# pzou01/unitree-rl-gym

Measured on AMD Instinct MI355X. Metric: env-steps/sec + PPO-iter wall-time, Go2 4096 envs/GPU at 1/2/4/8 MI355X, higher is better.
Workload: dtype fp32 env step; bf16 MFMA policy GEMMs (fp32 accumulate); 1 GPU; Go2 flat terrain, 4096 envs/GPU, MLP actor-critic 512-256-128, PPO 24 steps x 5 epochs x 4 mini-batches; num_envs_per_gpu=4096, decimation=4, parallelism=dp1

## Files before the change

unitree-rl-gym_amd/csrc/leggedsim.hip:

```cpp
#include <hip/hip_runtime.h>

#include <algorithm>
#include <cfloat>
#include <cmath>
#include <cstdint>
#include <cstdio>
#include <cstdlib>
#include <cstring>
#include <string>
#include <vector>

#include "../../include/leggedsim.h"
#include "lgs_detmath.h"

#define LGS_NPHASE 32
#ifdef LGS_PHASE_STAMPS
__device__ unsigned long long* g_phase_buf;
#define STAMP(i)                                                                                 \
    do {                                                                                         \
        __builtin_amdgcn_sched_barrier(0);                                                       \
        unsigned long long _t;                                                                   \
        asm volatile("s_memtime %0\n\ts_waitcnt lgkmcnt(0)" : "=s"(_t)::"memory");             \
        __builtin_amdgcn_sched_barrier(0);                                                       \
        if (threadIdx.x == 0) {                                                                  \
            if ((i) > 0) s.stamps[(i)] += _t - s.tlast;                                          \
            s.tlast = _t;                                                                        \
        }                                                                                        \
    } while (0)
#define STAMP_FLUSH(e)                                                                           \
    do {                                                                                         \
        if (threadIdx.x < LGS_NPHASE && g_phase_buf)                                             \
            g_phase_buf[(size_t)(e) * LGS_NPHASE + threadIdx.x] = s.stamps[threadIdx.x];         \
    } while (0)
#define STAMP_INIT()                                                                             \
    do {                                                                                         \
        if (threadIdx.x < LGS_NPHASE) s.stamps[threadIdx.x] = 0;                                 \
        if (threadIdx.x == 0) {                                                                  \
            s.stamps[18] = _wt0; s.stamps[20] = _wr0;                                            \
            s.stamps[22] = _whw; s.stamps[23] = _wxcc;                                           \
        }                                                                                        \
    } while (0)
#define STAMP_BEGIN()                                                                            \
    unsigned long long _wt0, _wr0;                                                               \
    unsigned _whw, _wxcc;                                                                        \
    asm volatile("s_memtime %0\n\ts_memrealtime %1\n\ts_getreg_b32 %2, hwreg(HW_REG_HW_ID)\n\t"   \
                 "s_getreg_b32 %3, hwreg(HW_REG_XCC_ID)\n\ts_waitcnt lgkmcnt(0)"                    \
                 : "=s"(_wt0), "=s"(_wr0), "=s"(_whw), "=s"(_wxcc)::"memory")
#define STAMP_END()                                                                              \
    do {                                                                                         \
        unsigned long long _t, _r;                                                               \
        asm volatile("s_memtime %0\n\ts_memrealtime %1\n\ts_waitcnt lgkmcnt(0)"                    \
                     : "=s"(_t), "=s"(_r)::"memory");                                            \
        if (threadIdx.x == 0) { s.stamps[19] = _t; s.stamps[21] = _r; }                          \
    } while (0)
#else
#define STAMP_BEGIN() do {} while (0)
#define STAMP_END() do {} while (0)
#define STAMP(i) do {} while (0)
#define STAMP_FLUSH(e) do {} while (0)
#define STAMP_INIT() do {} while (0)
#endif
#ifndef LGS_WAVES_PER_EU
#define LGS_WAVES_PER_EU 4
#endif
#ifndef LGS_WAVES_PER_EU_48
#define LGS_WAVES_PER_EU_48 3
#endif
#define MAXB LGS_MAX_BODIES
#define MAXD LGS_MAX_DEPTH
#define LGS_MAX_CHUNKS 32
#define LGS_PREFILTER_MARGIN 1e-3f
#define WAVE 64
// ... 3 lines not shown
static int set_err(int code, const std::string& msg) {
    g_err = msg;
    return code;
}
#define HIP_TRY(x)                                                                        \
    do {                                                                                  \
        hipError_t _e = (x);                                                              \
        if (_e != hipSuccess) return set_err(LGS_ERR_HIP, std::string(#x ": ") + hipGetErrorString(_e)); \
    } while (0)

struct DevModel {
    int B, D, P;
    int Br, Dr;
    const int* parent;
    const int* dof;
    const int* subtree_end;
    const int* depth;
    const int* chain;
    const float* joint_rot;
    const float* joint_pos;
    const float* axis;
    const float* mass;
    const float* com;
    const float* inertia;
    const float* dof_lower;
    const float* dof_upper;
    const float* dof_velocity;
    const int* pt_body;
    const float* pt_pos;
    const float* pt_radius;
    const float* bsph;
    const unsigned* chunk32;
    int nch32;
};

struct DevSim {
    float dt, gx, gy, gz;
    int iters;
    float contact_offset, rest_offset, max_depen, beta, ground_friction, armature;
    int clamp_qd, max_contacts, max_rows;
    const int16_t* hf;
    int hf_rows, hf_cols;
    float hf_inv_hs, hf_vs, hf_border;
    float hf_slope1, hf_nmin;
    const float4* selfp;
    int n_selfp, max_self;
    unsigned long long* stats;
};

__device__ __forceinline__ void count_drops(const DevSim& sp, int lane, int k, int v) {
    if (lane == 0 && v > 0) atomicAdd(sp.stats + LGS_NUM_CONTACT_STATS * (blockIdx.x & 7u) + k, (unsigned long long)v);
}

struct DevState {
    float* root;
    float* dofs;
    float* cforce;
    float* rbs;
    const float* friction;
    const float* added_mass;
    const float* torques_in;
    float* vsim;
    unsigned* pushed;
};

__device__ __forceinline__ float rl(float x, int l) {
// ... 138 lines not shown
    const float a = dot3(d1, d1), e = dot3(d2, d2), f = dot3(d2, r);
    const float eps = 1e-12f;
    float s, t;
    if (a <= eps && e <= eps) {
        s = 0.f; t = 0.f;
    } else if (a <= eps) {
        s = 0.f; t = clipf(f / e, 0.f, 1.f);
    } else {
        const float c = dot3(d1, r);
        if (e <= eps) {
            t = 0.f; s = clipf(-c / a, 0.f, 1.f);
        } else {
            const float b = dot3(d1, d2);
            const float den = a * e - b * b;
            s = den != 0.f ? clipf((b * f - c * e) / den, 0.f, 1.f) : 0.f;
            t = (b * s + f) / e;
            if (t < 0.f) { t = 0.f; s = clipf(-c / a, 0.f, 1.f); }
            else if (t > 1.f) { t = 1.f; s = clipf((b - c) / a, 0.f, 1.f); }
        }
    }
#pragma unroll
    for (int k = 0; k < 3; ++k) { c1[k] = p1[k] + d1[k] * s; c2[k] = p2[k] + d2[k] * t; }
}
__device__ __forceinline__ void self_tangents(const float* n, float* t1, float* t2) {
    float a0, a1, a2;
    if (fabsf(n[0]) < 0.57735f) { a0 = 1.f - n[0] * n[0]; a1 = 0.f - n[0] * n[1]; a2 = 0.f - n[0] * n[2]; }
    else { a0 = 0.f - n[1] * n[0]; a1 = 1.f - n[1] * n[1]; a2 = 0.f - n[1] * n[2]; }
    const float inv = 1.f / sqrtf(a0 * a0 + a1 * a1 + a2 * a2);
    t1[0] = a0 * inv; t1[1] = a1 * inv; t1[2] = a2 * inv;
    cross3(n, t1, t2);
}

template <int D, int B>
struct ModelCache {
    int dof[B], depth[B], se[B], dofbody[D > 0 ? D : 1];
    unsigned anc[D > 0 ? D : 1];
    unsigned char chain[B][MAXD];
    float jr[B][9], jp[B][3], ax[B][3], com[B][3], mass[B], in[B][6];
    float lo[D > 0 ? D : 1], hi[D > 0 ? D : 1], vl[D > 0 ? D : 1];
    float bs[B][5];
    unsigned ch32[LGS_MAX_CHUNKS];
};

template <int EPW, int D, int B>
__device__ __forceinline__ unsigned chunk_bodies(const ModelCache<D, B>& mc, int ch) {
    return EPW == 2 ? mc.ch32[ch] : (mc.ch32[2 * ch] | mc.ch32[2 * ch + 1]);
}

enum {
    MI_LIN_VEL = 0,
    MI_ANG_VEL = 3,
    MI_GRAVITY = 6,
    MI_PHASE = 9,
    MI_LEG_PHASE = 10,
    MI_CMD = 12,
    MI_CLEARANCE = 16,
    MI_FOOT_GROUND = 17,
    MI_COUNT = MI_FOOT_GROUND + LGS_MAX_FEET
};

template <int D, int B, int ROWS>
struct Smem {
    static constexpr int n = 6 + D;
    static constexpr int NP = (n % 2 == 0) ? n + 1 : n;
    static constexpr int AS = (ROWS % 2 == 0) ? ROWS + 1 : ROWS;
    static constexpr int EL = (D > LGS_MAX_CONTACT_BODIES ? D : LGS_MAX_CONTACT_BODIES) | 1;
    float root[16];
// ... 18 lines not shown
            float misc[32];
            static_assert(MI_COUNT <= 32, "misc holds every MI_* slot");
            float el[LGS_MAX_REWARDS][EL];
        } post;
        struct {
            int pwin[B];
            int sec_body[ROWS / 4];
            float sec[ROWS / 4][7];
            int sc_ab[ROWS / 4][2];
            float sc_tmp[ROWS / 4][7];
        } sel;
    } u;
    static constexpr int LP = (n + 3) / 4 * 4;
    __attribute__((aligned(16))) float L[n][LP];
    float Linv[n];
    float qf[n];
    float tgt[ROWS];
    int c_body[ROWS / 3];
    int c_body2[ROWS / 3];
    float c_pt[ROWS / 3][3];
    float c_fr[ROWS / 3][9];
    float c_sep[ROWS / 3];
    float cf[B][3];
    int flags[8];
    struct {
        long long ep;
        float cmd[4];
        float last_act[D > 0 ? D : 1], last_qd[D > 0 ? D : 1];
        float air[LGS_MAX_FEET];
        int lastc[LGS_MAX_FEET];
        float sums[LGS_MAX_REWARDS + 1];
        float kp[D > 0 ? D : 1], kd[D > 0 ? D : 1], strength[D > 0 ? D : 1];
        int delay;
    } pre;
#ifdef LGS_PHASE_STAMPS
    unsigned long long stamps[LGS_NPHASE];
    unsigned long long tlast;
#endif
};

template <int D, int B>
__device__ __forceinline__ void load_model(ModelCache<D, B>& c, const DevModel& md) {
    const int lane = threadIdx.x;
    if (lane < B) {
        const int j = md.dof[lane];
        c.dof[lane] = j;
        c.depth[lane] = md.depth[lane];
        c.se[lane] = md.subtree_end[lane];
        c.mass[lane] = md.mass[lane];
        if (j >= 0) c.dofbody[j] = lane;
    }
    for (int i = lane; i < B * MAXD; i += WAVE) (&c.chain[0][0])[i] = (unsigned char)md.chain[i];
    for (int i = lane; i < 9 * B; i += WAVE) (&c.jr[0][0])[i] = md.joint_rot[i];
    for (int i = lane; i < 3 * B; i += WAVE) {
        (&c.jp[0][0])[i] = md.joint_pos[i];
        (&c.ax[0][0])[i] = md.axis[i];
        (&c.com[0][0])[i] = md.com[i];
    }
    for (int i = lane; i < 6 * B; i += WAVE) (&c.in[0][0])[i] = md.inertia[i];
    for (int i = lane; i < 5 * B; i += WAVE) (&c.bs[0][0])[i] = md.bsph[i];
    if (lane < LGS_MAX_CHUNKS) c.ch32[lane] = lane < md.nch32 ? md.chunk32[lane] : 0u;
    if (lane < D) {
        int bj = 0;
        for (int b = 0; b < B; ++b) bj = md.dof[b] == lane ? b : bj;
        unsigned am = 0u;
        for (int b = 0; b <= bj; ++b) {
            const int i = md.dof[b];
            if (i >= 0 && i <= lane && bj < md.subtree_end[b]) am |= 1u << i;
        }
        c.anc[lane] = am;
        c.lo[lane] = md.dof_lower[lane];
        c.hi[lane] = md.dof_upper[lane];
        c.vl[lane] = md.dof_velocity[lane];
    }
}

template <int D, int CH>
__host__ __device__ constexpr bool l_nz(int i, int k) {
    return CH == 0 || k >= D || i >= D || i <= k + (D - 1 - k) % CH;
}

template <int D, int CH, int n, int LP>
__device__ __forceinline__ void uniform_back(const float* b, const float (*L)[LP], const float* Linv, float* xv) {
#pragma unroll
    for (int i = 0; i < n; ++i) xv[i] = b[i];
#pragma unroll
    for (int i = n - 1; i >= 0; --i) {
        float t = xv[i];
#pragma unroll
        for (int k = n - 1; k > i; --k)
            if (l_nz<D, CH>(k, i)) t = fmaf(-L[k][i], xv[k], t);
        xv[i] = t * Linv[i];
    }
}
template <int D, int CH, int n, int LP>
__device__ __forceinline__ void uniform_solve(const float* b, const float (*L)[LP], const float* Linv, float* xv) {
    float yv[n];
#pragma unroll
    for (int i = 0; i < n; ++i) {
        float t = b[i];
#pragma unroll
        for (int k = 0; k < i; ++k)
            if (l_nz<D, CH>(i, k)) t = fmaf(-L[i][k], yv[k], t);
        yv[i] = t * Linv[i];
    }
#pragma unroll
    for (int i = n - 1; i >= 0; --i) {
        float t = yv[i];
#pragma unroll
        for (int k = n - 1; k > i; --k)
            if (l_nz<D, CH>(k, i)) t = fmaf(-L[k][i], xv[k], t);
        xv[i] = t * Linv[i];
    }
}

template <int D, int B, int ROWS, int CH, int EPW, bool PAD = false>
__device__ void substep(Smem<D, B, ROWS>* sm, const ModelCache<D, B>& mc, const DevModel& md, const DevSim& sp,
                        float added_mass, float shape_mu, bool want_cf) {
    constexpr int n = 6 + D;
    Smem<D, B, ROWS>& s = sm[hh<EPW>()];
    int lane = hl<EPW>();
    asm volatile("" : "+v"(lane));
    const float dt = sp.dt;
    const float idt = 1.0f / dt;

    STAMP(0);
    if (lane < D) axis_angle(mc.ax[mc.dofbody[lane]], s.q[lane], s.u.fk.Ra[lane]);
    __syncthreads();
    if (lane < B) {
        float R[9], p[3], aw[3] = {0.f, 0.f, 0.f};
        quat_to_mat(s.root + 3, R);
        p[0] = s.root[0]; p[1] = s.root[1]; p[2] = s.root[2];
        const int d = mc.depth[lane];
        for (int l = 1; l <= d; ++l) {
            const int a = mc.chain[lane][l];
            float Rj[9], t[3];
            matmul(R, mc.jr[a], Rj);
            matvec(R, mc.jp[a], t);
            p[0] += t[0]; p[1] += t[1]; p[2] += t[2];
            const int j = mc.dof[a];
            if (j >= 0) {
                if (l == d) matvec(Rj, mc.ax[a], aw);
                matmul(Rj, s.u.fk.Ra[j], R);
            } else {
#pragma unroll
                for (int k = 0; k < 9; ++k) R[k] = Rj[k];
            }
        }
        float c[3];
        matvec(R, mc.com[lane], c);
#pragma unroll
        for (int k = 0; k < 9; ++k) s.R[lane][k] = R[k];
#pragma unroll
        for (int k = 0; k < 3; ++k) {
            s.p[lane][k] = p[k];
            s.aw[lane][k] = aw[k];
            s.cw[lane][k] = p[k] + c[k];
        }
    }
// ... 891 lines not shown
            matmul(R, mc.jr[a], Rj);
            matvec(R, mc.jp[a], tp);
            p[0] += tp[0]; p[1] += tp[1]; p[2] += tp[2];
            const int j = mc.dof[a];
            if (j >= 0) {
                matvec(Rj, mc.ax[a], aw);
                float Ra[9];
                axis_angle(mc.ax[a], s.q[j], Ra);
                matmul(Rj, Ra, R);
                const float qd = s.qd[j];
                float rp[3] = {p[0] - O[0], p[1] - O[1], p[2] - O[2]}, sv[3];
                cross3(rp, aw, sv);
#pragma unroll
                for (int k = 0; k < 3; ++k) { Vw[k] += aw[k] * qd; Vv[k] += sv[k] * qd; }
            } else {
#pragma unroll
                for (int k = 0; k < 9; ++k) R[k] = Rj[k];
            }
        }
        float c[3];
        matvec(R, mc.com[lane], c);
        float r[3] = {p[0] + c[0] - O[0], p[1] + c[1] - O[1], p[2] + c[2] - O[2]}, wr[3];
        cross3(Vw, r, wr);
        float* o = rbs_out + 13 * lane;
        o[0] = p[0]; o[1] = p[1]; o[2] = p[2];
        float qq[4];
        mat_to_quat(R, qq);
        o[3] = qq[0]; o[4] = qq[1]; o[5] = qq[2]; o[6] = qq[3];
#pragma unroll
        for (int k = 0; k < 3; ++k) { o[7 + k] = Vv[k] + wr[k]; o[10 + k] = Vw[k]; }
    }
}

template <int D, int B, int ROWS, int EPW, bool PAD = false>
__device__ __forceinline__ void load_state(Smem<D, B, ROWS>& s, const DevState& st, const DevModel& md, int e) {
    const int Dr = PAD ? md.Dr : D;
    const int lane = hl<EPW>();
    if (lane < 13) s.root[lane] = st.root[13 * e + lane];
    if (lane < 2 * D) {
        const float v = lane < 2 * Dr ? st.dofs[(size_t)2 * Dr * e + lane] : 0.f;
        if (lane & 1) s.qd[lane >> 1] = v; else s.q[lane >> 1] = v;
    }
}
template <int D, int B, int ROWS, int EPW, bool PAD = false>
__device__ __forceinline__ void store_state(Smem<D, B, ROWS>& s, const DevState& st, const DevModel& md, int e) {
    int lane = hl<EPW>();
    asm volatile("" : "+v"(lane));
    if (lane < 13) st.root[13 * e + lane] = s.root[lane];
    const int Dr = PAD ? md.Dr : D, Br = PAD ? md.Br : B;
    if (lane < 2 * Dr) st.dofs[(size_t)2 * Dr * e + lane] = (lane & 1) ? s.qd[lane >> 1] : s.q[lane >> 1];
    for (int i = lane; i < 3 * Br; i += WAVE / EPW) st.cforce[(size_t)3 * Br * e + i] = (&s.cf[0][0])[i];
}

template <int D, int B, int ROWS, int EPW, bool PAD = false>
__device__ __forceinline__ void load_post_inputs(Smem<D, B, ROWS>& s, const lgs_task_params& T,
                                                 const lgs_env_buffers& E, int N, int e, bool post) {
    const int lane = hl<EPW>();
    const int A = T.num_actions, Ad = PAD ? A : D, nf = T.num_feet;
    if (!post) {
        if (lane < Ad) s.pre.last_qd[lane] = E.last_dof_vel[Ad * e + lane];
        return;
    }
    const int nsum = T.num_rewards + (T.has_termination_reward ? 1 : 0);
    const float la = E.last_actions[A * e + (lane < A ? lane : 0)];
    const float lq = E.last_dof_vel[Ad * e + (lane < Ad ? lane : 0)];
    const float cm = E.commands[4 * e + (lane & 3)];
    const float su = E.episode_sums[(size_t)(lane < nsum ? lane : 0) * N + e];
    const long long ep = E.episode_length[e];
    float air = 0.f;
    int lc = 0;
    if (nf > 0) {
        air = E.feet_air_time[nf * e + (lane < nf ? lane : 0)];
        lc = E.last_contacts[nf * e + (lane < nf ? lane : 0)];
    }
    if (lane < A) s.pre.last_act[lane] = la;
    if (lane < Ad) s.pre.last_qd[lane] = lq;
    if (lane < 4) s.pre.cmd[lane] = cm;
    if (lane < nsum) s.pre.sums[lane] = su;
    if (lane < nf) { s.pre.air[lane] = air; s.pre.lastc[lane] = lc; }
    if (lane == 0) s.pre.ep = ep;
}

template <int D, int B, int ROWS, int CH, bool PAD = false>
__global__ __launch_bounds__(WAVE) void k_simulate(DevModel md, DevSim sp, DevState st, int N) {
    __shared__ Smem<D, B, ROWS> s;
    __shared__ ModelCache<D, B> mc;
    const int e = xcd_env(blockIdx.x, gridDim.x);
    if (e >= N) return;
    load_model(mc, md);
    const int Dr = PAD ? md.Dr : D, Br = PAD ? md.Br : B;
    load_state<D, B, ROWS, 1, PAD>(s, st, md, e);
    if (threadIdx.x < D)
        s.tau[threadIdx.x] = threadIdx.x < Dr ? st.torques_in[(size_t)Dr * e + threadIdx.x] : 0.f;
    __syncthreads();
    substep<D, B, ROWS, CH, 1, PAD>(&s, mc, md, sp, st.added_mass ? st.added_mass[e] : 0.f, st.friction ? st.friction[e] : 1.f, true);
    store_state<D, B, ROWS, 1, PAD>(s, st, md, e);
    if (st.rbs) body_states<D, B, ROWS, 1>(s, mc, st.rbs + (size_t)13 * Br * e, Br);
}

template <int D, int B, int ROWS, int CH, bool PAD = false>
__global__ __launch_bounds__(WAVE) void k_fk(DevModel md, DevState st, int N) {
    __shared__ Smem<D, B, ROWS> s;
    __shared__ ModelCache<D, B> mc;
    const int e = xcd_env(blockIdx.x, gridDim.x);
    if (e >= N) return;
    load_model(mc, md);
    const int Br = PAD ? md.Br : B;
    load_state<D, B, ROWS, 1, PAD>(s, st, md, e);
    __syncthreads();
    body_states<D, B, ROWS, 1>(s, mc, st.rbs + (size_t)13 * Br * e, Br);
}

struct DevEnv {
// ... 255 lines not shown

struct TerrainTail {
    long long* levels;
    const long long* types;
    const float* origins;
    long long* level_sum;
    float* heights;
    float hf_hs;
    float hf_inv_hs, hf_vs, hf_border;
    const int16_t* hf;
    int hf_rows, hf_cols;
    int obs_scan;
    float obs_offset, obs_clip, obs_scale, obs_noise;
};
__device__ __forceinline__ const TerrainTail& terrain_tail(const lgs_task_params& T) {
    return *reinterpret_cast<const TerrainTail*>(&T + 1);
}
__global__ void k_set_terrain_tail(TerrainTail* dst, TerrainTail v) { *dst = v; }

struct ActuatorTail {
    float* kp_scale;
    float* kd_scale;
    float* strength;
    int* delay;
    int enabled, resample;
    float kp_lo, kp_hi, kd_lo, kd_hi, st_lo, st_hi;
    int dl_lo, dl_hi;
};
static_assert(sizeof(TerrainTail) % alignof(ActuatorTail) == 0, "ActuatorTail follows TerrainTail");
__device__ __forceinline__ const ActuatorTail& actuator_tail(const lgs_task_params& T) {
    return *reinterpret_cast<const ActuatorTail*>(&terrain_tail(T) + 1);
}

template <int D, int B, int ROWS, int EPW, bool PAD = false>
__device__ __forceinline__ void load_actuator(Smem<D, B, ROWS>& s, const lgs_task_params& T,
                                              const lgs_env_buffers& E, int e, bool post) {
    const int lane = hl<EPW>();
    const int A = T.num_actions;
    const ActuatorTail& X = actuator_tail(T);
    const int jd = lane < D ? lane : 0;
    float kp = T.p_gains[jd], kd = T.d_gains[jd], st = 1.f;
    int dl = 0;
    if (X.enabled) {
        const size_t r = (size_t)A * e + (lane < A ? lane : 0);
        const float ks = X.kp_scale[r], ds = X.kd_scale[r], m = X.strength[r];
        dl = X.delay[e];
        if (!post) {
            const float la = E.last_actions[r];
            if (lane < A) s.pre.last_act[lane] = la;
        }
        if (lane < A) { kp = (kp * ks) * m; kd = (kd * ds) * m; st = m; }
        if (PAD && lane >= A && lane < D) s.pre.last_act[lane] = 0.f;
    }
    if (lane < D) { s.pre.kp[lane] = kp; s.pre.kd[lane] = kd; s.pre.strength[lane] = st; }
    if (lane == 0) s.pre.delay = dl;
}

template <int EPW>
__device__ __forceinline__ void resample_actuator(const lgs_task_params& T, int e, uint32_t step) {
    const ActuatorTail& X = actuator_tail(T);
    if (!X.enabled || !X.resample) return;
    const int lane = hl<EPW>();
    const int A = T.num_actions;
    const uint64_t seed = T.seed;
    if (lane < A) {
        const size_t r = (size_t)A * e + lane;
        X.kp_scale[r] = rand_range(X.kp_lo, X.kp_hi, philox_uniform(seed, e, step, LGS_STREAM_ACTUATOR, lane));
        X.kd_scale[r] = rand_range(X.kd_lo, X.kd_hi, philox_uniform(seed, e, step, LGS_STREAM_ACTUATOR, LGS_MAX_DOFS + lane));
        X.strength[r] = rand_range(X.st_lo, X.st_hi, philox_uniform(seed, e, step, LGS_STREAM_ACTUATOR, 2 * LGS_MAX_DOFS + lane));
    }
    if (lane == 0) {
        const int n = X.dl_hi - X.dl_lo + 1;
        X.delay[e] = X.dl_lo + min((int)(philox_uniform(seed, e, step, LGS_STREAM_ACTUATOR, 3 * LGS_MAX_DOFS) * (float)n), n - 1);
    }
}
template <int EPW>
__device__ __forceinline__ void height_scan(const TerrainTail& sp, const lgs_task_params& T, const float* root,
                                            float* out) {
    const int lane = hl<EPW>();
    const int ny = T.num_height_y, P = T.num_height_x * ny;
    const float qz = root[5], qw = root[6];
    const float nq = sqrtf(qz * qz + qw * qw);
    const float z = qz / nq, w = qw / nq;
    const float c = w * w - z * z, sn = 2.f * w * z;
    const float bx = root[0], by = root[1];
    for (int k = lane; k < P; k += WAVE / EPW) {
        const int ix = k / ny, iy = k - ix * ny;
// ... 370 lines not shown
            rand_range(-T.max_push_vel_xy, T.max_push_vel_xy, philox_uniform(seed, e, step, LGS_STREAM_PUSH, lane));
    } else if (lane < 6) {
        E.last_root_vel[6 * e + lane] = s.root[7 + lane];
    }
    if (vsim && lane >= 2 && lane < 6) E.last_root_vel[6 * e + lane] = s.root[7 + lane];
}

enum { MODE_STEP = 0, MODE_PHYSICS = 1, MODE_POST = 2, MODE_POST_REWARDS = 3, MODE_POST_FINISH = 4,
       MODE_POST_PREPARE = 5, MODE_POST_TERM_REWARDS = 6 };
__host__ __device__ constexpr int mode_part(int mode) {
    return mode == MODE_POST_REWARDS ? PART_REWARDS
         : mode == MODE_POST_FINISH ? PART_FINISH
         : mode == MODE_POST_PREPARE ? PART_PREPARE
         : mode == MODE_POST_TERM_REWARDS ? PART_TERM_REWARDS : PART_ALL;
}

template <int D, int B, int ROWS, int CH, int EPW, int WPE = 0, bool PAD = false>
__global__ __launch_bounds__(WAVE) __attribute__((amdgpu_waves_per_eu(WPE > 0 ? WPE : (EPW == 2 ? 2 : (ROWS <= 32 ? LGS_WAVES_PER_EU : LGS_WAVES_PER_EU_48))))) void k_step(DevModel md, DevSim sp, DevState st, const lgs_task_params* __restrict__ Tp,
                                               lgs_env_buffers E, int N, uint32_t step, int mode) {
    STAMP_BEGIN();
    __shared__ Smem<D, B, ROWS> sm[EPW];
    __shared__ ModelCache<D, B> mc;
#ifndef LGS_PHASE_STAMPS
    static_assert(EPW != 2 || EPW * sizeof(Smem<D, B, ROWS>) + sizeof(ModelCache<D, B>) <= 20 * 1024,
                  "k_step: LDS per workgroup above 20 KB");
#endif
    if (E.step_counter) step = (uint32_t)*E.step_counter;
    if (blockIdx.x == 0 && threadIdx.x == 0 && st.pushed && mode != MODE_PHYSICS) st.pushed[2] = step;
    const int e = EPW * xcd_env(blockIdx.x, gridDim.x) + hh<EPW>();
    if (EPW * xcd_env(blockIdx.x, gridDim.x) >= N) return;
    Smem<D, B, ROWS>& s = sm[hh<EPW>()];
    const lgs_task_params& T = *Tp;
    const int lane = hl<EPW>();
    load_model(mc, md);
#ifdef LGS_DIAG_MULTISTEP
    const uint32_t step0 = step;
    for (int tt = 0; tt < LGS_DIAG_MULTISTEP; ++tt) {
    step = step0 + (uint32_t)tt;
    __syncthreads();
#endif
    load_state<D, B, ROWS, EPW, PAD>(s, st, md, e);
    load_post_inputs<D, B, ROWS, EPW, PAD>(s, T, E, N, e, mode != MODE_PHYSICS);
    const int A = T.num_actions;
    const int Ad = PAD ? A : D, Br = PAD ? md.Br : B;
    float* rbs = (T.write_body_states && st.rbs) ? st.rbs + (size_t)13 * Br * e : nullptr;
    STAMP_INIT();
    if (mode == MODE_STEP || mode == MODE_PHYSICS) {
        load_actuator<D, B, ROWS, EPW, PAD>(s, T, E, e, mode != MODE_PHYSICS);
        float a = 0.f;
        if (lane < A) {
            const float* ain = E.actions_in ? E.actions_in : E.actions;
            a = clipf(ain[A * e + lane], -T.clip_actions, T.clip_actions);
            E.actions[A * e + lane] = a;
            s.act[lane] = a;
        }
        const float am = st.added_mass ? st.added_mass[e] : 0.f;
        const float mu = st.friction ? st.friction[e] : 1.f;
        __syncthreads();
        float traw = 0.f;
        for (int it = 0; it < T.decimation; ++it) {
            if (lane < D) {
                const float as = (it < s.pre.delay ? s.pre.last_act[lane] : a) * T.action_scale;
                const float q = s.q[lane], qd = s.qd[lane];
                const float kp = s.pre.kp[lane], kd = s.pre.kd[lane];
                float t;
                if (T.control_type == 0 && T.clamp_pd_targets) {
                    const float tg = clipf(as + T.default_dof_pos[lane], T.pd_target_lower[lane], T.pd_target_upper[lane]);
                    t = kp * (tg - q) - kd * qd;
                }
                else if (T.control_type == 0) t = kp * (as + T.default_dof_pos[lane] - q) - kd * qd;
                else if (T.control_type == 1) {
                    const float lqd = lane < Ad ? s.pre.last_qd[lane] : 0.f;
                    t = kp * (as - qd) - kd * (qd - lqd) / sp.dt;
                }
                else t = as * s.pre.strength[lane];
                traw = t;
                s.tau[lane] = clipf(t, -T.torque_limits[lane], T.torque_limits[lane]);
            }
            __syncthreads();
#ifndef LGS_DIAG_IO_ONLY
            substep<D, B, ROWS, CH, EPW, PAD>(sm, mc, md, sp, am, mu, it == T.decimation - 1);
#else
            if (lane < 3 * B) (&s.cf[0][0])[lane] = 0.f;
#endif
        }
        STAMP(0);
        if (T.record_unclipped_torques) {
            __syncthreads();
            if (lane < D) s.tau[lane] = traw;
        }
        if (lane < Ad) E.torques[Ad * e + lane] = s.tau[lane];
        if (rbs) body_states<D, B, ROWS, EPW>(s, mc, rbs, Br, T.body_state_mask);
    } else {
        if (lane < A) s.act[lane] = E.actions[A * e + lane];
        if (lane < D) s.tau[lane] = lane < Ad ? E.torques[Ad * e + lane] : 0.f;
        for (int i = lane; i < 3 * B; i += WAVE / EPW)
            (&s.cf[0][0])[i] = i < 3 * Br ? st.cforce[(size_t)3 * Br * e + i] : 0.f;
    }
    __syncthreads();
    STAMP(15);
    if (mode != MODE_PHYSICS)
        post_physics<D, B, ROWS, EPW, PAD>(s, T, E, rbs, N, e, step, RESET_STEP, mode_part(mode), st.vsim, st.pushed);
    __syncthreads();
    STAMP(16);
    store_state<D, B, ROWS, EPW, PAD>(s, st, md, e);
    STAMP(17);
    STAMP_END();
    STAMP_FLUSH(e);
#ifdef LGS_DIAG_MULTISTEP
    }
// ... 48 lines not shown
        float m = E.ep_means[nsum];
        if (any) m = (float)*E.terrain_level_sum / (float)N;
        E.ep_means[nsum] = m;
        if (E.ep_snapshot) E.ep_snapshot[nsum] = m;
    }
    if (E.time_outs_carry && any)
        for (int e = t; e < N; e += blockDim.x) E.time_outs_carry[e] = E.time_out[e];
    __syncthreads();
    if (t <= nsum) E.episode_acc[t] = 0.f;
    if (E.episode_acc_next && t <= nsum) E.episode_acc_next[t] = 0.f;
    if (t == 0 && advance) pushed_flag[(step + 1u) & 1u] = 0u;
    if (t == 0 && E.step_counter && advance) *E.step_counter += 1;
}

__global__ void k_copy_rows(float* dst, const float* src, const int32_t* ids, int n, int width) {
    const int i = blockIdx.x * blockDim.x + threadIdx.x;
    const int row = i / width, col = i % width;
    if (row >= n) return;
    const size_t r = (size_t)ids[row];
    dst[r * width + col] = src[r * width + col];
}

struct Inst;
struct Kernels;
struct lgs_sim {
    int N, B, D, P;
    const Inst* inst = nullptr;
    const Kernels* kern = nullptr;
    int device;
    hipStream_t stream = nullptr;
    DevModel md{};
    DevSim sp{};
    void* model_mem = nullptr;
    float* friction = nullptr;
    float* added_mass = nullptr;
    float* vsim = nullptr;
    unsigned* pushed = nullptr;
    unsigned long long* stats = nullptr;
    float* root = nullptr;
    float* dofs = nullptr;
    float* cforce = nullptr;
    float* rbs = nullptr;
    const float* torques = nullptr;
    lgs_task_params* task_dev = nullptr;
    int16_t* hf_mem = nullptr;
    float4* self_mem = nullptr;
    int has_task = 0;
    int task_curriculum = 0, task_heights = 0;
    int task_obs = 0, task_priv = 0, task_layout = 0, task_actions = 0, task_scan = 0;
    lgs_height_obs hobs{};
    float hf_hs = 0.f;
    TerrainTail tail_host{};
    lgs_actuator_rand act{};
    int task_decimation = 0;
    int epw = 1;
    std::vector<std::string> body_names, dof_names;
};

#define LGS_ROBOT_SHAPES X(12, 13, 6) X(10, 11, 5) X(12, 19, 3)

#ifndef LGS_EXTRA_SHAPES
#define LGS_EXTRA_SHAPES X(23, 24)
#endif
#ifndef LGS_GENERIC_SHAPES
#define LGS_GENERIC_SHAPES X(16, 24) X(26, 32)
#endif

enum Fit {
    FIT_EXACT,
    FIT_BODIES,
    FIT_DOFS
};

struct Kernels {
    using Step = void (*)(DevModel, DevSim, DevState, const lgs_task_params*, lgs_env_buffers, int, uint32_t, int);
    Step step;
    Step step_small;
    Step step2;
    void (*simulate)(DevModel, DevSim, DevState, int);
    void (*fk)(DevModel, DevState, int);
    void (*reset_all)(DevModel, DevState, const lgs_task_params*, lgs_env_buffers, int, uint32_t, const uint8_t*);
};
template <int D, int B, int ROWS, int CH, bool PAD, bool EPW2>
static Kernels kernels_of() {
    Kernels k{};
    k.step = k_step<D, B, ROWS, CH, 1, PAD ? 2 : 0, PAD>;
    if constexpr (EPW2) k.step2 = k_step<D, B, ROWS, CH, 2, 0, PAD>;
    else if constexpr (!PAD) k.step_small = k_step<D, B, ROWS, CH, 1, 4, PAD>;
    k.simulate = k_simulate<D, B, ROWS, CH, PAD>;
    k.fk = k_fk<D, B, ROWS, CH, PAD>;
    k.reset_all = k_reset_all<D, B, ROWS, CH, PAD>;
    return k;
}

struct Inst {
    int Dt, Bt;
    int rows;
    int chain;
    Fit fit;
    bool epw2;
    Kernels chained, dense;
    bool takes(int D, int B) const {
        return fit == FIT_DOFS ? D <= Dt && B + (Dt - D) <= Bt : D == Dt && (fit == FIT_BODIES ? B <= Bt : B == Bt);
    }
};
template <int D, int B, int ROWS, int CH, Fit FIT, bool EPW2>
static Inst inst_of() {
    constexpr bool PAD = FIT != FIT_EXACT;
    return {D, B, ROWS, CH, FIT, EPW2, kernels_of<D, B, ROWS, CH, PAD, EPW2>(), kernels_of<D, B, ROWS, 0, PAD, EPW2>()};
}
static const Inst g_insts[] = {
#define X(D_, B_, CH_) inst_of<D_, B_, 32, CH_, FIT_EXACT, true>(),
    LGS_ROBOT_SHAPES
#undef X
#define X(D_, B_, CH_) inst_of<D_, B_, 48, CH_, FIT_EXACT, false>(),
    LGS_ROBOT_SHAPES
#undef X
#define X(D_, B_) inst_of<D_, B_, 48, 0, FIT_BODIES, false>(),
    LGS_EXTRA_SHAPES
#undef X
#define X(D_, B_) inst_of<D_, B_, 48, 0, FIT_DOFS, false>(),
    LGS_GENERIC_SHAPES
#undef X
};
// ... 136 lines not shown
    for (int b = B; b < Bt; ++b) bsph[(size_t)5 * b + 3] = -1.f;
    size_t ints = (size_t)Bt * (4 + LGS_MAX_DEPTH) + (size_t)P + chunk32.size();
    size_t floats = (size_t)Bt * (9 + 3 + 3 + 1 + 3 + 6 + 5) + (size_t)Dt * 3 + (size_t)P * 4;
    size_t bytes = ints * 4 + floats * 4 + 512;
    HIP_TRY(hipMalloc(&s->model_mem, bytes));
    char* host = (char*)calloc(1, bytes);
    size_t off = 0;
    auto put = [&](const void* src, size_t n) -> size_t {
        size_t o = off;
        if (n) memcpy(host + off, src, n);
        off += (n + 15) & ~size_t(15);
        return o;
    };
    size_t o_parent = put(parent.data(), 4 * Bt), o_dof = put(dofv.data(), 4 * Bt), o_se = put(se.data(), 4 * Bt);
    size_t o_depth = put(depth.data(), 4 * Bt), o_chain = put(chain.data(), 4 * Bt * LGS_MAX_DEPTH);
    size_t o_jr = put(jr.data(), 36 * Bt), o_jp = put(jp.data(), 12 * Bt), o_ax = put(ax.data(), 12 * Bt);
    size_t o_mass = put(mass.data(), 4 * Bt), o_com = put(com.data(), 12 * Bt), o_in = put(inertia.data(), 24 * Bt);
    size_t o_lo = put(dlo.data(), 4 * Dt), o_hi = put(dhi.data(), 4 * Dt), o_vel = put(dvel.data(), 4 * Dt);
    size_t o_pb = put(m->pt_body, 4 * P), o_pp = put(m->pt_pos, 12 * P), o_pr = put(m->pt_radius, 4 * P);
    size_t o_bs = put(bsph.data(), 20 * Bt), o_ch = put(chunk32.data(), 4 * chunk32.size());
    if (off > bytes) { free(host); return set_err(LGS_ERR_STATE, "model packing overflow"); }
    HIP_TRY(hipMemcpy(s->model_mem, host, off, hipMemcpyHostToDevice));
    free(host);
    char* d = (char*)s->model_mem;
    DevModel& md = s->md;
    md.B = Bt; md.D = Dt; md.P = P; md.Br = B; md.Dr = D;
    md.parent = (const int*)(d + o_parent); md.dof = (const int*)(d + o_dof); md.subtree_end = (const int*)(d + o_se);
    md.depth = (const int*)(d + o_depth); md.chain = (const int*)(d + o_chain);
    md.joint_rot = (const float*)(d + o_jr); md.joint_pos = (const float*)(d + o_jp); md.axis = (const float*)(d + o_ax);
    md.mass = (const float*)(d + o_mass); md.com = (const float*)(d + o_com); md.inertia = (const float*)(d + o_in);
    md.dof_lower = (const float*)(d + o_lo); md.dof_upper = (const float*)(d + o_hi); md.dof_velocity = (const float*)(d + o_vel);
    md.pt_body = (const int*)(d + o_pb); md.pt_pos = (const float*)(d + o_pp); md.pt_radius = (const float*)(d + o_pr);
    md.bsph = (const float*)(d + o_bs); md.chunk32 = (const unsigned*)(d + o_ch); md.nch32 = nch32;
    DevSim& sp = s->sp;
    sp.dt = p->dt; sp.gx = p->gravity[0]; sp.gy = p->gravity[1]; sp.gz = p->gravity[2];
    sp.iters = p->solver_iterations; sp.contact_offset = p->contact_offset; sp.rest_offset = p->rest_offset;
    sp.max_depen = p->max_depenetration_velocity; sp.beta = p->baumgarte; sp.ground_friction = p->ground_friction;
    sp.armature = p->armature; sp.clamp_qd = p->clamp_joint_velocity; sp.max_contacts = p->max_contacts;
    sp.max_rows = p->max_rows;
    sp.hf = nullptr; sp.hf_rows = sp.hf_cols = 0; sp.hf_inv_hs = sp.hf_vs = sp.hf_border = 0.f;
    sp.hf_slope1 = 1.f; sp.hf_nmin = 1.f;
    sp.selfp = nullptr; sp.n_selfp = 0; sp.max_self = 0;
    HIP_TRY(hipMalloc(&s->friction, sizeof(float) * num_envs));
    HIP_TRY(hipMalloc(&s->added_mass, sizeof(float) * num_envs));
    HIP_TRY(hipMalloc(&s->vsim, sizeof(float) * 2 * num_envs));
    HIP_TRY(hipMalloc(&s->pushed, sizeof(unsigned) * 3));
    HIP_TRY(hipMemset(s->pushed, 0, sizeof(unsigned) * 3));
    HIP_TRY(hipMalloc(&s->stats, sizeof(unsigned long long) * 8 * LGS_NUM_CONTACT_STATS));
    HIP_TRY(hipMemset(s->stats, 0, sizeof(unsigned long long) * 8 * LGS_NUM_CONTACT_STATS));
    s->sp.stats = s->stats;
    HIP_TRY(hipMemset(s->added_mass, 0, sizeof(float) * num_envs));
    {
        float* ones = (float*)malloc(sizeof(float) * num_envs);
        for (int i = 0; i < num_envs; ++i) ones[i] = p->ground_friction;
        HIP_TRY(hipMemcpy(s->friction, ones, sizeof(float) * num_envs, hipMemcpyHostToDevice));
        free(ones);
    }
    static_assert(sizeof(lgs_task_params) % alignof(TerrainTail) == 0, "TerrainTail follows lgs_task_params");
    HIP_TRY(hipMalloc(&s->task_dev, sizeof(lgs_task_params) + sizeof(TerrainTail) + sizeof(ActuatorTail)));
    HIP_TRY(hipMemset(s->task_dev, 0, sizeof(lgs_task_params) + sizeof(TerrainTail) + sizeof(ActuatorTail)));
    *out = s;
    return LGS_OK;
}

LGS_API int lgs_destroy_sim(lgs_sim* s) {
    if (!s) return LGS_OK;
    (void)hipFree(s->model_mem);
    (void)hipFree(s->friction);
    (void)hipFree(s->added_mass);
    (void)hipFree(s->vsim);
    (void)hipFree(s->pushed);
    (void)hipFree(s->stats);
    (void)hipFree(s->task_dev);
    (void)hipFree(s->hf_mem);
    (void)hipFree(s->self_mem);
    delete s;
    return LGS_OK;
}

LGS_API int lgs_set_heightfield(lgs_sim* s, const int16_t* heights, int32_t rows, int32_t cols,
                                float horizontal_scale, float vertical_scale, float border_size) {
    if (!s) return set_err(LGS_ERR_ARG, "null sim");
    if (heights && rows > 0 && (rows < 2 || cols < 2 || !(horizontal_scale > 0.f) || !(vertical_scale > 0.f)))
        return set_err(LGS_ERR_ARG, "lgs_set_heightfield: need rows, cols >= 2 and positive scales");
    HIP_TRY(hipStreamSynchronize(s->stream));
    (void)hipFree(s->hf_mem);
    s->hf_mem = nullptr;
    s->sp.hf = nullptr;
    s->sp.hf_rows = s->sp.hf_cols = 0;
    if (!heights || rows <= 0) return LGS_OK;
    const size_t bytes = sizeof(int16_t) * (size_t)rows * (size_t)cols;
    HIP_TRY(hipMalloc(&s->hf_mem, bytes));
    HIP_TRY(hipMemcpy(s->hf_mem, heights, bytes, hipMemcpyHostToDevice));
    s->sp.hf = s->hf_mem;
    s->sp.hf_rows = rows; s->sp.hf_cols = cols;
    s->sp.hf_inv_hs = 1.0f / horizontal_scale;
    s->hf_hs = horizontal_scale;
    s->sp.hf_vs = vertical_scale;
    s->sp.hf_border = border_size;
    double g2 = 0.0;
// ... 435 lines not shown
```

Before: 12.84 million env-steps/s.

## Prebuild model cache image and issue all per-env global loads before committing to LDS

Builds the per-model shared-memory cache once at sim creation into a flat global image, so each kernel block copies it with coalesced 16-byte loads instead of gathering many scattered model arrays. State, post-input, actuator, action, mass and friction loads are split into issue/commit phases so all global reads are in flight together before any are written to LDS, hiding latency at step start. Per-joint default pos, torque limits and PD target bounds are staged into shared memory so the decimation loop no longer rereads them from global parameters. The cost is more register pressure from values held across the issue phase, plus an extra image buffer and init kernel.

New measurement: 13.03 million env-steps/s, median of 6. +1.5%, better.

```diff
diff --git a/unitree-rl-gym_amd/csrc/leggedsim.hip b/unitree-rl-gym_amd/csrc/leggedsim.hip
--- a/unitree-rl-gym_amd/csrc/leggedsim.hip
+++ b/unitree-rl-gym_amd/csrc/leggedsim.hip
@@ -38,6 +38,7 @@
         if (threadIdx.x == 0) {                                                                  \
             s.stamps[18] = _wt0; s.stamps[20] = _wr0;                                            \
             s.stamps[22] = _whw; s.stamps[23] = _wxcc;                                           \
+            s.tlast = _wt0;                                                                      \
         }                                                                                        \
     } while (0)
 #define STAMP_BEGIN()                                                                            \
@@ -107,6 +108,7 @@
     const float* bsph;
     const unsigned* chunk32;
     int nch32;
+    const uint4* image;
 };
 
 struct DevSim {
@@ -311,7 +313,7 @@
 }
 
 template <int D, int B>
-struct ModelCache {
+struct alignas(16) ModelCache {
     int dof[B], depth[B], se[B], dofbody[D > 0 ? D : 1];
     unsigned anc[D > 0 ? D : 1];
     unsigned char chain[B][MAXD];
@@ -396,6 +398,7 @@
         float sums[LGS_MAX_REWARDS + 1];
         float kp[D > 0 ? D : 1], kd[D > 0 ? D : 1], strength[D > 0 ? D : 1];
         int delay;
+        float dflt[D > 0 ? D : 1], tlim[D > 0 ? D : 1], tg_lo[D > 0 ? D : 1], tg_hi[D > 0 ? D : 1];
     } pre;
 #ifdef LGS_PHASE_STAMPS
     unsigned long long stamps[LGS_NPHASE];
@@ -404,7 +407,39 @@
 };
 
 template <int D, int B>
+struct ModelWords {
+    static constexpr int NV = sizeof(ModelCache<D, B>) / 16, K = (NV + WAVE - 1) / WAVE;
+    static_assert(sizeof(ModelCache<D, B>) % 16 == 0, "the image is copied in 16-byte words");
+    typedef unsigned word __attribute__((ext_vector_type(4)));
+    word v[K];
+};
+template <int D, int B>
+__device__ __forceinline__ ModelWords<D, B> load_model_issue(const DevModel& md) {
+    ModelWords<D, B> w;
+    using word = typename ModelWords<D, B>::word;
+    const auto* image = (const __attribute__((address_space(1))) word*)md.image;
+#pragma unroll
+    for (int k = 0; k < w.K; ++k) {
+        const int i = (int)threadIdx.x + WAVE * k;
+        w.v[k] = image[i < w.NV ? i : 0];
+    }
+    return w;
+}
+template <int D, int B>
+__device__ __forceinline__ void load_model_commit(ModelCache<D, B>& c, const ModelWords<D, B>& w) {
+#pragma unroll
+    for (int k = 0; k < w.K; ++k) {
+        const int i = (int)threadIdx.x + WAVE * k;
+        if (i < w.NV) reinterpret_cast<typename ModelWords<D, B>::word*>(&c)[i] = w.v[k];
+    }
+}
+template <int D, int B>
 __device__ __forceinline__ void load_model(ModelCache<D, B>& c, const DevModel& md) {
+    load_model_commit(c, load_model_issue<D, B>(md));
+}
+
+template <int D, int B>
+__device__ __forceinline__ void build_model(ModelCache<D, B>& c, const DevModel& md) {
     const int lane = threadIdx.x;
     if (lane < B) {
         const int j = md.dof[lane];
@@ -438,6 +473,16 @@
         c.vl[lane] = md.dof_velocity[lane];
     }
 }
+template <int D, int B>
+__global__ __launch_bounds__(WAVE) void k_model_image(DevModel md, uint4* out) {
+    __shared__ ModelCache<D, B> mc;
+    constexpr int NV = ModelWords<D, B>::NV;
+    for (int i = threadIdx.x; i < NV; i += WAVE) reinterpret_cast<uint4*>(&mc)[i] = make_uint4(0u, 0u, 0u, 0u);
+    __syncthreads();
+    build_model(mc, md);
+    __syncthreads();
+    for (int i = threadIdx.x; i < NV; i += WAVE) out[i] = reinterpret_cast<const uint4*>(&mc)[i];
+}
 
 template <int D, int CH>
 __host__ __device__ constexpr bool l_nz(int i, int k) {
@@ -488,7 +533,7 @@
     const float dt = sp.dt;
     const float idt = 1.0f / dt;
 
-    STAMP(0);
+    STAMP(30);
     if (lane < D) axis_angle(mc.ax[mc.dofbody[lane]], s.q[lane], s.u.fk.Ra[lane]);
     __syncthreads();
     if (lane < B) {
@@ -1446,15 +1491,31 @@
     }
 }
 
+struct StateRegs { float root, qv; };
+template <int D, int EPW, bool PAD = false>
+__device__ __forceinline__ StateRegs load_state_issue(const DevState& st, const DevModel& md, int e) {
+    const int Dr = PAD ? md.Dr : D;
+    const int lane = hl<EPW>();
+    asm volatile("" : "+v"(e));
+    StateRegs r;
+    r.root = st.root[13 * e + (lane < 13 ? lane : 0)];
+    const float* pq = Dr > 0 ? st.dofs + ((size_t)2 * Dr * e + (lane < 2 * Dr ? lane : 0)) : st.root + 13 * e;
+    r.qv = *pq;
+    return r;
+}
+template <int D, int B, int ROWS, int EPW, bool PAD = false>
+__device__ __forceinline__ void load_state_commit(Smem<D, B, ROWS>& s, const DevModel& md, const StateRegs& r) {
+    const int Dr = PAD ? md.Dr : D;
+    const int lane = hl<EPW>();
+    if (lane < 13) s.root[lane] = r.root;
+    if (lane < 2 * D) {
+        const float v = lane < 2 * Dr ? r.qv : 0.f;
+        if (lane & 1) s.qd[lane >> 1] = v; else s.q[lane >> 1] = v;
+    }
+}
 template <int D, int B, int ROWS, int EPW, bool PAD = false>
 __device__ __forceinline__ void load_state(Smem<D, B, ROWS>& s, const DevState& st, const DevModel& md, int e) {
-    const int Dr = PAD ? md.Dr : D;
-    const int lane = hl<EPW>();
-    if (lane < 13) s.root[lane] = st.root[13 * e + lane];
-    if (lane < 2 * D) {
-        const float v = lane < 2 * Dr ? st.dofs[(size_t)2 * Dr * e + lane] : 0.f;
-        if (lane & 1) s.qd[lane >> 1] = v; else s.q[lane >> 1] = v;
-    }
+    load_state_commit<D, B, ROWS, EPW, PAD>(s, md, load_state_issue<D, EPW, PAD>(st, md, e));
 }
 template <int D, int B, int ROWS, int EPW, bool PAD = false>
 __device__ __forceinline__ void store_state(Smem<D, B, ROWS>& s, const DevState& st, const DevModel& md, int e) {
@@ -1466,33 +1527,45 @@
     for (int i = lane; i < 3 * Br; i += WAVE / EPW) st.cforce[(size_t)3 * Br * e + i] = (&s.cf[0][0])[i];
 }
 
-template <int D, int B, int ROWS, int EPW, bool PAD = false>
-__device__ __forceinline__ void load_post_inputs(Smem<D, B, ROWS>& s, const lgs_task_params& T,
-                                                 const lgs_env_buffers& E, int N, int e, bool post) {
+struct PostRegs {
+    float la, lq, cm, su, air;
+    long long ep;
+    int lc;
+};
+template <int D, int EPW, bool PAD = false>
+__device__ __forceinline__ PostRegs load_post_inputs_issue(const lgs_task_params& T, const lgs_env_buffers& E, int N,
+                                                           int e, bool post) {
     const int lane = hl<EPW>();
     const int A = T.num_actions, Ad = PAD ? A : D, nf = T.num_feet;
-    if (!post) {
-        if (lane < Ad) s.pre.last_qd[lane] = E.last_dof_vel[Ad * e + lane];
-        return;
-    }
+    asm volatile("" : "+v"(e));
+    PostRegs r{};
+    r.lq = E.last_dof_vel[Ad * e + (lane < Ad ? lane : 0)];
+    if (!post) return r;
     const int nsum = T.num_rewards + (T.has_termination_reward ? 1 : 0);
-    const float la = E.last_actions[A * e + (lane < A ? lane : 0)];
-    const float lq = E.last_dof_vel[Ad * e + (lane < Ad ? lane : 0)];
-    const float cm = E.commands[4 * e + (lane & 3)];
-    const float su = E.episode_sums[(size_t)(lane < nsum ? lane : 0) * N + e];
-    const long long ep = E.episode_length[e];
-    float air = 0.f;
-    int lc = 0;
-    if (nf > 0) {
-        air = E.feet_air_time[nf * e + (lane < nf ? lane : 0)];
-        lc = E.last_contacts[nf * e + (lane < nf ? lane : 0)];
-    }
-    if (lane < A) s.pre.last_act[lane] = la;
-    if (lane < Ad) s.pre.last_qd[lane] = lq;
-    if (lane < 4) s.pre.cmd[lane] = cm;
-    if (lane < nsum) s.pre.sums[lane] = su;
-    if (lane < nf) { s.pre.air[lane] = air; s.pre.lastc[lane] = lc; }
-    if (lane == 0) s.pre.ep = ep;
+    const int fi = nf * e + (lane < nf ? lane : 0);
+    const float* pa = nf > 0 ? E.feet_air_time + fi : E.commands + 4 * e;
+    const uint8_t* pc = nf > 0 ? E.last_contacts + fi : reinterpret_cast<const uint8_t*>(E.commands + 4 * e);
+    r.air = *pa;
+    r.lc = *pc;
+    r.la = E.last_actions[A * e + (lane < A ? lane : 0)];
+    r.cm = E.commands[4 * e + (lane & 3)];
+    r.su = E.episode_sums[(size_t)(lane < nsum ? lane : 0) * N + e];
+    r.ep = E.episode_length[e];
+    return r;
+}
+template <int D, int B, int ROWS, int EPW, bool PAD = false>
+__device__ __forceinline__ void load_post_inputs_commit(Smem<D, B, ROWS>& s, const lgs_task_params& T,
+                                                        const PostRegs& r, bool post) {
+    const int lane = hl<EPW>();
+    const int A = T.num_actions, Ad = PAD ? A : D, nf = T.num_feet;
+    if (lane < Ad) s.pre.last_qd[lane] = r.lq;
+    if (!post) return;
+    const int nsum = T.num_rewards + (T.has_termination_reward ? 1 : 0);
+    if (lane < A) s.pre.last_act[lane] = r.la;
+    if (lane < 4) s.pre.cmd[lane] = r.cm;
+    if (lane < nsum) s.pre.sums[lane] = r.su;
+    if (lane < nf) { s.pre.air[lane] = r.air; s.pre.lastc[lane] = r.lc; }
+    if (lane == 0) s.pre.ep = r.ep;
 }
 
 template <int D, int B, int ROWS, int CH, bool PAD = false>
@@ -1814,27 +1887,47 @@
     return *reinterpret_cast<const ActuatorTail*>(&terrain_tail(T) + 1);
 }
 
-template <int D, int B, int ROWS, int EPW, bool PAD = false>
-__device__ __forceinline__ void load_actuator(Smem<D, B, ROWS>& s, const lgs_task_params& T,
-                                              const lgs_env_buffers& E, int e, bool post) {
+struct ActuatorRegs {
+    float kp, kd, ks, ds, m, la, dflt, tlim, tg_lo, tg_hi;
+    int dl;
+};
+template <int D, int EPW>
+__device__ __forceinline__ ActuatorRegs load_actuator_issue(const lgs_task_params& T, const lgs_env_buffers& E, int e,
+                                                            bool post) {
     const int lane = hl<EPW>();
     const int A = T.num_actions;
     const ActuatorTail& X = actuator_tail(T);
     const int jd = lane < D ? lane : 0;
-    float kp = T.p_gains[jd], kd = T.d_gains[jd], st = 1.f;
-    int dl = 0;
+    ActuatorRegs a{};
+    a.kp = T.p_gains[jd]; a.kd = T.d_gains[jd];
+    a.dflt = T.default_dof_pos[jd]; a.tlim = T.torque_limits[jd];
+    a.tg_lo = T.pd_target_lower[jd]; a.tg_hi = T.pd_target_upper[jd];
     if (X.enabled) {
         const size_t r = (size_t)A * e + (lane < A ? lane : 0);
-        const float ks = X.kp_scale[r], ds = X.kd_scale[r], m = X.strength[r];
-        dl = X.delay[e];
-        if (!post) {
-            const float la = E.last_actions[r];
-            if (lane < A) s.pre.last_act[lane] = la;
-        }
-        if (lane < A) { kp = (kp * ks) * m; kd = (kd * ds) * m; st = m; }
+        a.ks = X.kp_scale[r]; a.ds = X.kd_scale[r]; a.m = X.strength[r];
+        a.dl = X.delay[e];
+        if (!post) a.la = E.last_actions[r];
+    }
+    return a;
+}
+template <int D, int B, int ROWS, int EPW, bool PAD = false>
+__device__ __forceinline__ void load_actuator_commit(Smem<D, B, ROWS>& s, const lgs_task_params& T,
+                                                     const ActuatorRegs& a, bool post) {
+    const int lane = hl<EPW>();
+    const int A = T.num_actions;
+    float kp = a.kp, kd = a.kd, st = 1.f;
+    int dl = 0;
+    if (actuator_tail(T).enabled) {
+        dl = a.dl;
+        if (!post && lane < A) s.pre.last_act[lane] = a.la;
+        if (lane < A) { kp = (kp * a.ks) * a.m; kd = (kd * a.ds) * a.m; st = a.m; }
         if (PAD && lane >= A && lane < D) s.pre.last_act[lane] = 0.f;
     }
-    if (lane < D) { s.pre.kp[lane] = kp; s.pre.kd[lane] = kd; s.pre.strength[lane] = st; }
+    if (lane < D) {
+        s.pre.kp[lane] = kp; s.pre.kd[lane] = kd; s.pre.strength[lane] = st;
+        s.pre.dflt[lane] = a.dflt; s.pre.tlim[lane] = a.tlim;
+        s.pre.tg_lo[lane] = a.tg_lo; s.pre.tg_hi[lane] = a.tg_hi;
+    }
     if (lane == 0) s.pre.delay = dl;
 }
 
@@ -2271,31 +2364,46 @@
     Smem<D, B, ROWS>& s = sm[hh<EPW>()];
     const lgs_task_params& T = *Tp;
     const int lane = hl<EPW>();
-    load_model(mc, md);
+    const bool phys = mode == MODE_STEP || mode == MODE_PHYSICS;
+    constexpr bool HOLD_MODEL = ModelWords<D, B>::K <= 4;
+    ModelWords<D, B> mw;
+    if constexpr (HOLD_MODEL) mw = load_model_issue<D, B>(md);
+    else load_model(mc, md);
 #ifdef LGS_DIAG_MULTISTEP
     const uint32_t step0 = step;
     for (int tt = 0; tt < LGS_DIAG_MULTISTEP; ++tt) {
     step = step0 + (uint32_t)tt;
     __syncthreads();
 #endif
-    load_state<D, B, ROWS, EPW, PAD>(s, st, md, e);
-    load_post_inputs<D, B, ROWS, EPW, PAD>(s, T, E, N, e, mode != MODE_PHYSICS);
     const int A = T.num_actions;
     const int Ad = PAD ? A : D, Br = PAD ? md.Br : B;
+    const StateRegs sr = load_state_issue<D, EPW, PAD>(st, md, e);
+    const PostRegs pr = load_post_inputs_issue<D, EPW, PAD>(T, E, N, e, mode != MODE_PHYSICS);
+    ActuatorRegs ar{};
+    float ain = 0.f, am = 0.f, mu = 1.f;
+    if (phys) {
+        ar = load_actuator_issue<D, EPW>(T, E, e, mode != MODE_PHYSICS);
+        ain = (E.actions_in ? E.actions_in : E.actions)[A * e + (lane < A ? lane : 0)];
+        am = *(st.added_mass ? st.added_mass + e : st.root + 13 * e);
+        mu = *(st.friction ? st.friction + e : st.root + 13 * e);
+    }
+    if constexpr (HOLD_MODEL) load_model_commit(mc, mw);
+    load_state_commit<D, B, ROWS, EPW, PAD>(s, md, sr);
+    load_post_inputs_commit<D, B, ROWS, EPW, PAD>(s, T, pr, mode != MODE_PHYSICS);
     float* rbs = (T.write_body_states && st.rbs) ? st.rbs + (size_t)13 * Br * e : nullptr;
     STAMP_INIT();
-    if (mode == MODE_STEP || mode == MODE_PHYSICS) {
-        load_actuator<D, B, ROWS, EPW, PAD>(s, T, E, e, mode != MODE_PHYSICS);
+    if (phys) {
+        load_actuator_commit<D, B, ROWS, EPW, PAD>(s, T, ar, mode != MODE_PHYSICS);
         float a = 0.f;
         if (lane < A) {
-            const float* ain = E.actions_in ? E.actions_in : E.actions;
-            a = clipf(ain[A * e + lane], -T.clip_actions, T.clip_actions);
+            a = clipf(ain, -T.clip_actions, T.clip_actions);
             E.actions[A * e + lane] = a;
             s.act[lane] = a;
         }
-        const float am = st.added_mass ? st.added_mass[e] : 0.f;
-        const float mu = st.friction ? st.friction[e] : 1.f;
+        if (!st.added_mass) am = 0.f;
+        if (!st.friction) mu = 1.f;
         __syncthreads();
+        STAMP(29);
         float traw = 0.f;
         for (int it = 0; it < T.decimation; ++it) {
             if (lane < D) {
@@ -2304,17 +2412,17 @@
                 const float kp = s.pre.kp[lane], kd = s.pre.kd[lane];
                 float t;
                 if (T.control_type == 0 && T.clamp_pd_targets) {
-                    const float tg = clipf(as + T.default_dof_pos[lane], T.pd_target_lower[lane], T.pd_target_upper[lane]);
+                    const float tg = clipf(as + s.pre.dflt[lane], s.pre.tg_lo[lane], s.pre.tg_hi[lane]);
                     t = kp * (tg - q) - kd * qd;
                 }
-                else if (T.control_type == 0) t = kp * (as + T.default_dof_pos[lane] - q) - kd * qd;
+                else if (T.control_type == 0) t = kp * (as + s.pre.dflt[lane] - q) - kd * qd;
                 else if (T.control_type == 1) {
                     const float lqd = lane < Ad ? s.pre.last_qd[lane] : 0.f;
                     t = kp * (as - qd) - kd * (qd - lqd) / sp.dt;
                 }
                 else t = as * s.pre.strength[lane];
                 traw = t;
-                s.tau[lane] = clipf(t, -T.torque_limits[lane], T.torque_limits[lane]);
+                s.tau[lane] = clipf(t, -s.pre.tlim[lane], s.pre.tlim[lane]);
             }
             __syncthreads();
 #ifndef LGS_DIAG_IO_ONLY
@@ -2429,6 +2537,7 @@
     DevModel md{};
     DevSim sp{};
     void* model_mem = nullptr;
+    uint4* image_mem = nullptr;
     float* friction = nullptr;
     float* added_mass = nullptr;
     float* vsim = nullptr;
@@ -2477,6 +2586,8 @@
     void (*simulate)(DevModel, DevSim, DevState, int);
     void (*fk)(DevModel, DevState, int);
     void (*reset_all)(DevModel, DevState, const lgs_task_params*, lgs_env_buffers, int, uint32_t, const uint8_t*);
+    void (*model_image)(DevModel, uint4*);
+    size_t image_bytes;
 };
 template <int D, int B, int ROWS, int CH, bool PAD, bool EPW2>
 static Kernels kernels_of() {
@@ -2487,6 +2598,8 @@
     k.simulate = k_simulate<D, B, ROWS, CH, PAD>;
     k.fk = k_fk<D, B, ROWS, CH, PAD>;
     k.reset_all = k_reset_all<D, B, ROWS, CH, PAD>;
+    k.model_image = k_model_image<D, B>;
+    k.image_bytes = sizeof(ModelCache<D, B>);
     return k;
 }
 
@@ -2689,6 +2802,12 @@
     md.dof_lower = (const float*)(d + o_lo); md.dof_upper = (const float*)(d + o_hi); md.dof_velocity = (const float*)(d + o_vel);
     md.pt_body = (const int*)(d + o_pb); md.pt_pos = (const float*)(d + o_pp); md.pt_radius = (const float*)(d + o_pr);
     md.bsph = (const float*)(d + o_bs); md.chunk32 = (const unsigned*)(d + o_ch); md.nch32 = nch32;
+    HIP_TRY(hipMalloc(&s->image_mem, s->kern->image_bytes));
+    md.image = nullptr;
+    hipLaunchKernelGGL(s->kern->model_image, dim3(1), dim3(WAVE), 0, nullptr, md, s->image_mem);
+    HIP_TRY(hipGetLastError());
+    HIP_TRY(hipStreamSynchronize(nullptr));
+    md.image = s->image_mem;
     DevSim& sp = s->sp;
     sp.dt = p->dt; sp.gx = p->gravity[0]; sp.gy = p->gravity[1]; sp.gz = p->gravity[2];
     sp.iters = p->solver_iterations; sp.contact_offset = p->contact_offset; sp.rest_offset = p->rest_offset;
@@ -2723,6 +2842,7 @@
 LGS_API int lgs_destroy_sim(lgs_sim* s) {
     if (!s) return LGS_OK;
     (void)hipFree(s->model_mem);
+    (void)hipFree(s->image_mem);
     (void)hipFree(s->friction);
     (void)hipFree(s->added_mass);
     (void)hipFree(s->vsim);
```
